# AnyiRao/video_unscreen

Measured on NVIDIA B200. Metric: frames/sec at 1080p & 4K (1/2/4/8 B200) + % HBM roofline vs host-CPU ref, higher is better.
Workload: dtype u8

## Files before the change

video_unscreen_b200/csrc/vu_median_sad.cuh:

```cuda
#pragma once
#include <cuda.h>
#include <cuda_runtime.h>
#include <stdint.h>

#include <type_traits>
#include "vu_tma.cuh"

namespace vu {
namespace msad {

__device__ __forceinline__ unsigned sad_acc(unsigned a, unsigned b, unsigned c) {
  unsigned d;
  asm("vabsdiff4.u32.u32.u32.add %0, %1, %2, %3;" : "=r"(d) : "r"(a), "r"(b), "r"(c));
  return d;
}

template <int G>
__device__ __forceinline__ void transpose_groups(unsigned (&d)[4 * G]) {
#pragma unroll
  for (int g = 0; g < G; ++g) {
    const unsigned a = d[4 * g], b = d[4 * g + 1], c = d[4 * g + 2], e = d[4 * g + 3];
    const unsigned ab_lo = __byte_perm(a, b, 0x5140), ab_hi = __byte_perm(a, b, 0x7362);
    const unsigned ce_lo = __byte_perm(c, e, 0x5140), ce_hi = __byte_perm(c, e, 0x7362);
    d[4 * g] = __byte_perm(ab_lo, ce_lo, 0x5410);
    d[4 * g + 1] = __byte_perm(ab_lo, ce_lo, 0x7632);
    d[4 * g + 2] = __byte_perm(ab_hi, ce_hi, 0x5410);
    d[4 * g + 3] = __byte_perm(ab_hi, ce_hi, 0x7632);
  }
}

template <int GI>
__device__ __forceinline__ unsigned ldg_strided(const uint8_t* base, unsigned stride) {
  unsigned long long addr;
  unsigned v;
  asm("mad.wide.u32 %0, %1, %2, %3;" : "=l"(addr) : "r"(stride), "n"(GI), "l"(base));
  asm volatile("ld.global.nc.u32 %0, [%1];" : "=r"(v) : "l"(addr));
  return v;
}

template <int I, int N, class F>
__device__ __forceinline__ void static_for(F&& f) {
  if constexpr (I < N) {
    f(std::integral_constant<int, I>{});
    static_for<I + 1, N>(f);
  }
}

constexpr unsigned BIG = 0x7fffffffu;
constexpr unsigned FULL = 0xffffffffu;

template <int SPLIT, int G, bool RANGE>
__device__ __forceinline__ void eval_s(const unsigned (&d)[4 * G], const int (&m)[4], int delta, unsigned (&S)[4]) {
  constexpr int LPS = 32 / SPLIT;
  unsigned q[4], s[4];
#pragma unroll
  for (int j = 0; j < 4; ++j) {
    q[j] = (unsigned)(RANGE ? min(max(m[j], 0), 255) : m[j]) * 0x01010101u;
    s[j] = 0;
  }
#pragma unroll
  for (int g = 0; g < G; ++g) {
#pragma unroll
    for (int j = 0; j < 4; ++j) s[j] = sad_acc(d[4 * g + j], q[j], s[j]);
  }
#pragma unroll
  for (int j = 0; j < 4; ++j) {
#pragma unroll
    for (int o = LPS; o < 32; o <<= 1) s[j] += __shfl_xor_sync(FULL, s[j], o);
    s[j] += (unsigned)(delta * m[j]);
    S[j] = (RANGE && (m[j] < 0 || m[j] > 255)) ? BIG : s[j];
  }
}

template <int SPLIT, int G, bool RANGE>
__device__ __forceinline__ void fib_search(const unsigned (&d)[4 * G], int delta, int k0, int fa, int fb, int fc, int (&a)[4], int (&r)[4],
                                           unsigned (&smin)[4], unsigned (&sl)[4], unsigned (&sr)[4]) {
  unsigned S1[4], S2[4];
  {
    int i1[4], i2[4];
#pragma unroll
    for (int j = 0; j < 4; ++j) {
      i1[j] = a[j] + fb;
      i2[j] = a[j] + fa;
      sl[j] = sr[j] = BIG;
    }
    eval_s<SPLIT, G, RANGE>(d, i1, delta, S1);
    eval_s<SPLIT, G, RANGE>(d, i2, delta, S2);
  }
#pragma unroll 1
  for (int k = k0; k >= 5; --k) {
    int nidx[4];
    bool left[4];
#pragma unroll
    for (int j = 0; j < 4; ++j) {
      left[j] = S1[j] <= S2[j];
      if (left[j]) {
        sr[j] = S2[j];
        S2[j] = S1[j];
        nidx[j] = a[j] + fc;
      } else {
        sl[j] = S1[j];
        a[j] += fb;
        S1[j] = S2[j];
        nidx[j] = a[j] + fb;
      }
    }
    unsigned Sn[4];
    eval_s<SPLIT, G, RANGE>(d, nidx, delta, Sn);
#pragma unroll
    for (int j = 0; j < 4; ++j) {
      if (left[j]) S1[j] = Sn[j];
      else S2[j] = Sn[j];
    }
    const int t = fb - fc;
    fa = fb;
    fb = fc;
    fc = t;
  }
#pragma unroll
  for (int j = 0; j < 4; ++j) {
    if (S1[j] <= S2[j]) {
      r[j] = a[j] + 1;
      smin[j] = S1[j];
      sr[j] = S2[j];
    } else {
      r[j] = a[j] + 2;
      smin[j] = S2[j];
      sl[j] = S1[j];
    }
  }
}

template <int SPLIT, int G, int SS>
__device__ __forceinline__ unsigned sad_median(const unsigned (&d)[4 * G], int n, int delta) {
  int a[4], r[4];
  unsigned smin[4], sl[4], sr[4];
  bool full = (SS == 0);
  if (SS > 0) {
    constexpr int EPP = 4 / SPLIT;
    const int part = (threadIdx.x & 31) / (32 / SPLIT);
    unsigned smp[EPP][4];
#pragma unroll
    for (int e = 0; e < EPP; ++e)
#pragma unroll
      for (int t = 0; t < 4; ++t) {
        unsigned v = d[4 * (t * SS) + e];
#pragma unroll
        for (int p = 1; p < SPLIT; ++p) v = (part == p) ? d[4 * (t * SS) + p * EPP + e] : v;
        smp[e][t] = v;
      }
    int est[EPP];
#pragma unroll
    for (int e = 0; e < EPP; ++e) est[e] = 0;
#pragma unroll 1
    for (int bit = 128; bit > 0; bit >>= 1) {
#pragma unroll
      for (int e = 0; e < EPP; ++e) {
        const unsigned q1 = (unsigned)(est[e] | bit) * 0x01010101u, q0 = q1 - 0x01010101u;
        unsigned s0 = 0, s1 = 0;
#pragma unroll
        for (int t = 0; t < 4; ++t) {
          s0 = sad_acc(smp[e][t], q0, s0);
          s1 = sad_acc(smp[e][t], q1, s1);
        }
        if (s1 < s0) est[e] |= bit;
      }
    }
#pragma unroll
    for (int j = 0; j < 4; ++j) {
      const int c = __shfl_sync(FULL, est[j % EPP], (j / EPP) * (32 / SPLIT) + (threadIdx.x & (32 / SPLIT - 1)));
      a[j] = min(max(c - 10, -1), 235);
    }
    fib_search<SPLIT, G, false>(d, delta, 8, 13, 8, 5, a, r, smin, sl, sr);
    bool fail = false;
#pragma unroll
    for (int j = 0; j < 4; ++j) fail |= (sl[j] == BIG && r[j] > 0) || (sr[j] == BIG && r[j] < 255);
    full = __any_sync(FULL, fail);
  }
  if (full) {
#pragma unroll
    for (int j = 0; j < 4; ++j) a[j] = -1;
    fib_search<SPLIT, G, true>(d, delta, 14, 233, 144, 89, a, r, smin, sl, sr);
  }
  int lo[4], hi[4];
#pragma unroll
  for (int j = 0; j < 4; ++j) lo[j] = hi[j] = r[j];
  if (!(n & 1)) {
    bool openL[4], openR[4];
    bool any = false;
#pragma unroll
    for (int j = 0; j < 4; ++j) {
      openL[j] = openR[j] = false;
      if (sl[j] == smin[j]) { lo[j] = r[j] - 1; openL[j] = lo[j] > 0; }
      if (sr[j] == smin[j]) { hi[j] = r[j] + 1; openR[j] = hi[j] < 255; }
      any |= openL[j] | openR[j];
    }
#pragma unroll 1
    for (int it = 0; it < 4 && __any_sync(FULL, any); ++it) {
      int idx[4];
      unsigned S[4];
#pragma unroll
      for (int j = 0; j < 4; ++j) idx[j] = openL[j] ? lo[j] - 1 : (openR[j] ? hi[j] + 1 : r[j]);
      eval_s<SPLIT, G, false>(d, idx, delta, S);
      any = false;
#pragma unroll
      for (int j = 0; j < 4; ++j) {
        if (openL[j]) {
          if (S[j] == smin[j]) { --lo[j]; openL[j] = lo[j] > 0; }
          else openL[j] = false;
        } else if (openR[j]) {
          if (S[j] == smin[j]) { ++hi[j]; openR[j] = hi[j] < 255; }
          else openR[j] = false;
        }
        any |= openL[j] | openR[j];
      }
    }
    if (__any_sync(FULL, any)) {
      int L[4], R[4];
#pragma unroll
      for (int j = 0; j < 4; ++j) { R[j] = lo[j]; L[j] = openL[j] ? 0 : lo[j]; }
      while (__any_sync(FULL, (L[0] < R[0]) | (L[1] < R[1]) | (L[2] < R[2]) | (L[3] < R[3]))) {
        int idx[4];
        unsigned S[4];
#pragma unroll
        for (int j = 0; j < 4; ++j) idx[j] = (L[j] + R[j]) >> 1;
        eval_s<SPLIT, G, false>(d, idx, delta, S);
#pragma unroll
        for (int j = 0; j < 4; ++j)
          if (L[j] < R[j]) {
            const int mid = (L[j] + R[j]) >> 1;
            if (S[j] == smin[j]) R[j] = mid;
            else L[j] = mid + 1;
          }
      }
#pragma unroll
      for (int j = 0; j < 4; ++j) { lo[j] = R[j]; L[j] = hi[j]; R[j] = openR[j] ? 255 : hi[j]; }
      while (__any_sync(FULL, (L[0] < R[0]) | (L[1] < R[1]) | (L[2] < R[2]) | (L[3] < R[3]))) {
        int idx[4];
        unsigned S[4];
#pragma unroll
        for (int j = 0; j < 4; ++j) idx[j] = (L[j] + R[j] + 1) >> 1;
        eval_s<SPLIT, G, false>(d, idx, delta, S);
#pragma unroll
        for (int j = 0; j < 4; ++j)
          if (L[j] < R[j]) {
            const int mid = (L[j] + R[j] + 1) >> 1;
            if (S[j] == smin[j]) L[j] = mid;
            else R[j] = mid - 1;
          }
      }
#pragma unroll
      for (int j = 0; j < 4; ++j) hi[j] = L[j];
    }
  }
  unsigned res = 0;
#pragma unroll
  for (int j = 0; j < 4; ++j) res |= (unsigned)((lo[j] + hi[j]) >> 1) << (8 * j);
  return res;
}

template <int SPLIT>
__device__ __forceinline__ bool pad_high(int part) { return SPLIT == 2 ? part == 1 : (part == 1 || part == 2); }

template <int SPLIT, int G, int GFULL, int SS, int CTAS>
__global__ void __launch_bounds__(128, CTAS) median_sad_kernel(const uint8_t* __restrict__ frames, uint8_t* __restrict__ out, int n, long long m,
                                                               int nseg, unsigned zero) {
  constexpr int LPS = 32 / SPLIT;
  constexpr int SEG = LPS * 4;
  const int lane = threadIdx.x & 31, warp = threadIdx.x >> 5;
  const int part = lane / LPS, li = lane % LPS;
  const int seg = blockIdx.x * 4 + warp;
  if (seg >= nseg) return;
  const int cnt0 = (n + SPLIT - 1) / SPLIT;
  const int cnt = (n - part + SPLIT - 1) / SPLIT;
  const int Q = (cnt0 + 3) >> 2;
  const unsigned pad = pad_high<SPLIT>(part) ? 0xFFFFFFFFu : 0u;
  int n0 = 0, n255 = 0;
#pragma unroll
  for (int p = 0; p < SPLIT; ++p) {
    const int c = 4 * G - (n - p + SPLIT - 1) / SPLIT;
    if (pad_high<SPLIT>(p)) n255 += c;
    else n0 += c;
  }
  const int delta = n255 - n0;
  unsigned gstride[4];
  const uint8_t* rowbase[4];
#pragma unroll
  for (int r = 0; r < 4; ++r) {
    rowbase[r] = frames + (long long)seg * SEG + li * 4 + ((long long)SPLIT * (r * Q) + part) * m;
    gstride[r] = (unsigned)(SPLIT * m) + (unsigned)r * zero;
  }
  unsigned d[4 * G];
  static_for<0, G>([&](auto gi) {
    constexpr int g = decltype(gi)::value;
#pragma unroll
    for (int r = 0; r < 4; ++r) {
      const bool ok = (r < 3 && g < GFULL) ? true : (g < Q && r * Q + g < cnt);
      d[4 * g + r] = pad;
      if (ok) d[4 * g + r] = ldg_strided<g>(rowbase[r], gstride[r]);
    }
  });
  transpose_groups<G>(d);
  const unsigned res = sad_median<SPLIT, G, SS>(d, n, delta);
  if (part == 0) reinterpret_cast<unsigned*>(out + (long long)seg * SEG)[li] = res;
}


using tma::mbar_expect_tx;
using tma::mbar_init;
using tma::mbar_wait;
__device__ __forceinline__ void tma_load_2d(unsigned dst, const void* tmap, int c0, int c1, unsigned mbar) { tma::load_2d(dst, tmap, c0, c1, mbar); }

template <int SPLIT, int G, int GQ, int SS, int WARPS, int CTAS>
__global__ void __launch_bounds__(WARPS * 32, CTAS) median_sad_tma_kernel(const __grid_constant__ CUtensorMap tmap, uint8_t* __restrict__ out, int n,
                                                                          int ntiles) {
  extern __shared__ __align__(128) uint8_t smem_tma[];
  constexpr int LPS = 32 / SPLIT;
  constexpr int SEG = LPS * 4;
  constexpr int TILE = WARPS * SEG;
  constexpr int ROWS = SPLIT * 4 * G;
  constexpr unsigned BOX_BYTES = 4 * G * TILE;
  const int lane = threadIdx.x & 31, warp = threadIdx.x >> 5;
  const int part = lane / LPS, li = lane % LPS;
  const int cnt0 = (n + SPLIT - 1) / SPLIT;
  const int Q = (cnt0 + 3) >> 2;
  const int delta = -(ROWS - n);
  uint64_t* mbar_p = reinterpret_cast<uint64_t*>(smem_tma + ROWS * TILE);
  unsigned* count_p = reinterpret_cast<unsigned*>(mbar_p + 1);
  const unsigned mbar = (unsigned)__cvta_generic_to_shared(mbar_p);
  const unsigned sdata = (unsigned)__cvta_generic_to_shared(smem_tma);
  auto fetch = [&](int tile) {
    mbar_expect_tx(mbar, SPLIT * BOX_BYTES);
#pragma unroll
    for (int b = 0; b < SPLIT; ++b) tma_load_2d(sdata + b * BOX_BYTES, &tmap, tile * (TILE > 256 ? TILE / 4 : TILE), b * 4 * G, mbar);
  };
  if (threadIdx.x == 0) {
    mbar_init(mbar, 1);
    *count_p = 0;
    asm volatile("fence.mbarrier_init.release.cluster;" ::: "memory");
  }
  __syncthreads();
  int tile = blockIdx.x;
  if (threadIdx.x == 0 && tile < ntiles) fetch(tile);
  const uint8_t* rowaddr[4];
#pragma unroll
  for (int r = 0; r < 4; ++r) rowaddr[r] = smem_tma + (SPLIT * (r * Q) + part) * TILE + warp * SEG + li * 4;
  unsigned parity = 0;
  for (; tile < ntiles; tile += gridDim.x) {
    mbar_wait(mbar, parity);
    parity ^= 1;
    unsigned d[4 * G];
#pragma unroll
    for (int g = 0; g < G; ++g) {
#pragma unroll
      for (int r = 0; r < 4; ++r) {
        d[4 * g + r] = 0;
        if (g < GQ || g < Q) d[4 * g + r] = *reinterpret_cast<const unsigned*>(rowaddr[r] + g * (SPLIT * TILE));
      }
    }
    transpose_groups<G>(d);
    __syncwarp();
    if (lane == 0) {
      __threadfence_block();
      const unsigned old = atomicAdd(count_p, 1u);
      if (old % WARPS == WARPS - 1 && tile + (int)gridDim.x < ntiles) {
        __threadfence_block();
        asm volatile("fence.proxy.async.shared::cta;" ::: "memory");
        fetch(tile + gridDim.x);
      }
    }
    const unsigned res = sad_median<SPLIT, G, SS>(d, n, delta);
    if (part == 0) reinterpret_cast<unsigned*>(out + ((long long)tile * WARPS + warp) * SEG)[li] = res;
  }
}

constexpr int RF_WARPS = 8, RF_ROWS = 64, RF_STAGES = 4, RF_PROBES = 8;
constexpr int RF_TILE = RF_WARPS * 64;
constexpr int RF_STAGE_BYTES = RF_ROWS * RF_TILE;
constexpr int RF_SMEM = RF_STAGES * RF_STAGE_BYTES + RF_STAGES * 16;

__global__ void __launch_bounds__(RF_WARPS * 32, 1) median_refine_kernel(const __grid_constant__ CUtensorMap tmap, uint8_t* __restrict__ out,
                                                                         uint8_t* __restrict__ flags, int n, int ntiles, int nchunks) {
  extern __shared__ __align__(128) uint8_t smem_rf[];
  const int lane = threadIdx.x & 31, warp = threadIdx.x >> 5;
  const int part = lane >> 4, li = lane & 15;
  uint64_t* mbar_p = reinterpret_cast<uint64_t*>(smem_rf + RF_STAGES * RF_STAGE_BYTES);
  unsigned* count_p = reinterpret_cast<unsigned*>(mbar_p + RF_STAGES);
  const unsigned mbar0 = (unsigned)__cvta_generic_to_shared(mbar_p);
  const unsigned sdata = (unsigned)__cvta_generic_to_shared(smem_rf);
  const int my_tiles = blockIdx.x < ntiles ? (ntiles - 1 - (int)blockIdx.x) / (int)gridDim.x + 1 : 0;
  const int J = my_tiles * nchunks;
  auto issue = [&](int j) {
    const int tile = blockIdx.x + (j / nchunks) * gridDim.x, chunk = j % nchunks, st = j % RF_STAGES;
    mbar_expect_tx(mbar0 + 8 * st, RF_STAGE_BYTES);
    tma_load_2d(sdata + st * RF_STAGE_BYTES, &tmap, tile * (RF_TILE / 4), chunk * RF_ROWS, mbar0 + 8 * st);
  };
  if (threadIdx.x == 0) {
    for (int st = 0; st < RF_STAGES; ++st) {
      mbar_init(mbar0 + 8 * st, 1);
      count_p[st] = 0;
    }
    asm volatile("fence.mbarrier_init.release.cluster;" ::: "memory");
  }
  __syncthreads();
  if (threadIdx.x == 0)
    for (int j = 0; j < RF_STAGES && j < J; ++j) issue(j);
  const int delta = -(nchunks * RF_ROWS - n);
  unsigned acc[RF_PROBES][4], q[RF_PROBES][4];
  int a0[4];
  const uint8_t* lane_row = smem_rf + part * RF_TILE + warp * 64 + li * 4;
  for (int j = 0; j < J; ++j) {
    const int tile = blockIdx.x + (j / nchunks) * gridDim.x, chunk = j % nchunks, st = j % RF_STAGES;
    const int64_t seg = (int64_t)tile * RF_WARPS + warp;
    if (chunk == 0) {
      const unsigned e = *reinterpret_cast<const unsigned*>(out + seg * 64 + li * 4);
#pragma unroll
      for (int k = 0; k < 4; ++k) {
        a0[k] = min(max((int)((e >> (8 * k)) & 255u) - 4, 0), 256 - RF_PROBES);
#pragma unroll
        for (int p = 0; p < RF_PROBES; ++p) {
          q[p][k] = (unsigned)(a0[k] + p) * 0x01010101u;
          acc[p][k] = 0u;
        }
      }
    }
// ... 57 lines not shown
```

video_unscreen_b200/csrc/vu_temporal.cu:

```cuda
#include <cstdlib>

#include "vu_common.cuh"
#include "vu_median_sad.cuh"

namespace vu {
namespace {

constexpr int WARPS = 7;
constexpr int MTHREADS = WARPS * 32;
constexpr int BIN_STRIDE = WARPS * 128;
constexpr int HIST_BYTES = 256 * BIN_STRIDE;

struct PolU16x2 {
  static constexpr int PX = 2;
  __device__ static __forceinline__ void add(unsigned char* base, unsigned w) {
#pragma unroll
    for (int j = 0; j < 2; ++j) atomicAdd(reinterpret_cast<unsigned*>(base + ((w >> (8 * j)) & 0xFFu) * BIN_STRIDE), 1u << (16 * j));
  }
  __device__ static __forceinline__ void unpack(unsigned w, unsigned* c) { c[0] = w & 0xFFFFu; c[1] = w >> 16; }
};

template <int PX>
__device__ __forceinline__ unsigned load_px(const uint8_t* p) {
  if (PX == 4) return __ldg(reinterpret_cast<const unsigned*>(p));
// ... 65 lines not shown
#pragma unroll
      for (int b = 0; b < 16; ++b) {
        unsigned t[PX];
        P::unpack(*reinterpret_cast<unsigned*>(base + (g * 16 + b) * BIN_STRIDE), t);
#pragma unroll
        for (int j = 0; j < PX; ++j) c[j] += t[j];
      }
#pragma unroll
      for (int j = 0; j < PX; ++j) {
        const unsigned nc = cum[j] + c[j];
        if (nc <= klo) { gsel[j][0] = g + 1; before[j][0] = nc; }
        if (nc <= khi) { gsel[j][1] = g + 1; before[j][1] = nc; }
        cum[j] = nc;
      }
    }
    unsigned res = 0;
#pragma unroll
    for (int j = 0; j < PX; ++j) {
      unsigned med[2];
#pragma unroll
      for (int q = 0; q < 2; ++q) {
        const unsigned k = q ? khi : klo;
        if (q == 1 && khi == klo) { med[1] = med[0]; continue; }
        const unsigned g = min(gsel[j][q], 15u);
        unsigned v = g * 16, c2 = before[j][q];
#pragma unroll 4
        for (int b = 0; b < 16; ++b) {
          unsigned t[PX];
          P::unpack(*reinterpret_cast<unsigned*>(base + (g * 16 + b) * BIN_STRIDE), t);
          c2 += t[j];
          if (c2 <= k) v = g * 16 + b + 1;
        }
        med[q] = min(v, 255u);
      }
      res |= ((med[0] + med[1]) >> 1) << (8 * j);
    }
    uint8_t* dst = out + (long long)seg * SEG;
    if (PX == 4) reinterpret_cast<unsigned*>(dst)[lane] = res;
    else reinterpret_cast<unsigned short*>(dst)[lane] = (unsigned short)res;
    __syncwarp();
  }
}

template <int SPLIT, int G, int GFULL, int SS, int CTAS>
int launch_median_sad(const uint8_t* frames, int n, int64_t m, int64_t nseg, uint8_t* out, vu_stream_t stream) {
  msad::median_sad_kernel<SPLIT, G, GFULL, SS, CTAS><<<(unsigned)((nseg + 3) / 4), 128, 0, S(stream)>>>(frames, out, n, m, (int)nseg, 0u);
  note_launch();
  return record_cuda(cudaGetLastError());
}

using tma::encode_tiled_fn;
using tma::EncodeTiledFn;

template <int SPLIT, int G, int GQ, int SS, int TMA_WARPS, int TMA_CTAS>
int launch_median_sad_tma(const uint8_t* frames, int n, int64_t m, int64_t ntiles, uint8_t* out, vu_stream_t stream, int64_t pitch = 0) {
  if (pitch == 0) pitch = m;
  constexpr int TILE = TMA_WARPS * (128 / SPLIT);
  constexpr int SMEM = SPLIT * 4 * G * TILE + 16;
  constexpr bool U32 = TILE > 256;
  static_assert(TILE <= 1024 && 4 * G <= 256, "TMA box limits");
  EncodeTiledFn enc = encode_tiled_fn();
  if (!enc) return VU_ERR_UNSUPPORTED;
  CUtensorMap tmap;
  const cuuint64_t dims[2] = {(cuuint64_t)(U32 ? m / 4 : m), (cuuint64_t)n};
  const cuuint64_t strides[1] = {(cuuint64_t)pitch};
  const cuuint32_t box[2] = {(cuuint32_t)(U32 ? TILE / 4 : TILE), (cuuint32_t)(4 * G)};
  const cuuint32_t estr[2] = {1, 1};
  if (enc(&tmap, U32 ? CU_TENSOR_MAP_DATA_TYPE_UINT32 : CU_TENSOR_MAP_DATA_TYPE_UINT8, 2, const_cast<uint8_t*>(frames), dims, strides, box, estr, CU_TENSOR_MAP_INTERLEAVE_NONE,
          CU_TENSOR_MAP_SWIZZLE_NONE, CU_TENSOR_MAP_L2_PROMOTION_L2_256B, CU_TENSOR_MAP_FLOAT_OOB_FILL_NONE) != CUDA_SUCCESS)
    return VU_ERR_UNSUPPORTED;
  auto kernel = msad::median_sad_tma_kernel<SPLIT, G, GQ, SS, TMA_WARPS, TMA_CTAS>;
  static bool configured = false;
  if (!configured) {
    int e = record_cuda(cudaFuncSetAttribute(kernel, cudaFuncAttributeMaxDynamicSharedMemorySize, SMEM));
    if (e) return e;
    configured = true;
  }
  const int64_t cap = (int64_t)device_sms() * TMA_CTAS;
  const int grid = (int)(ntiles < cap ? ntiles : cap);
  kernel<<<grid, TMA_WARPS * 32, SMEM, S(stream)>>>(tmap, out, n, (int)ntiles);
  note_launch();
  return record_cuda(cudaGetLastError());
}

__global__ void __launch_bounds__(256) median_tail_kernel(const uint8_t* __restrict__ frames, uint8_t* __restrict__ out, int n, long long m,
                                                          long long first) {
  __shared__ unsigned hist[256];
  const long long e = first + blockIdx.x;
  hist[threadIdx.x] = 0;
  __syncthreads();
  for (int f = threadIdx.x; f < n; f += 256) atomicAdd(&hist[__ldg(frames + (long long)f * m + e)], 1u);
  __syncthreads();
  if (threadIdx.x == 0) {
    const unsigned klo = (unsigned)(n - 1) >> 1, khi = (unsigned)n >> 1;
    unsigned cum = 0, lo = 255, hi = 255;
    bool flo = false, fhi = false;
    for (int b = 0; b < 256; ++b) {
      cum += hist[b];
      if (!flo && cum > klo) { lo = b; flo = true; }
      if (!fhi && cum > khi) { hi = b; fhi = true; }
    }
    out[e] = (uint8_t)((lo + hi) >> 1);
  }
}

constexpr int TT = 256;
__global__ void __launch_bounds__(TT) masked_mean_kernel(const uint8_t* __restrict__ frames, const uint8_t* __restrict__ masks, int n,
                                                         int64_t ngroups, int64_t npix, int min_count, uint8_t* __restrict__ bg_out,
                                                         uint8_t* __restrict__ always_out) {
  const int64_t stride = (int64_t)gridDim.x * blockDim.x;
  for (int64_t g = (int64_t)blockIdx.x * blockDim.x + threadIdx.x; g < ngroups; g += stride) {
    unsigned sum[12], cnt[4];
#pragma unroll
    for (int i = 0; i < 12; ++i) sum[i] = 0;
#pragma unroll
    for (int i = 0; i < 4; ++i) cnt[i] = 0;
    const unsigned* f4 = reinterpret_cast<const unsigned*>(frames) + 3 * g;
    const unsigned* m4 = reinterpret_cast<const unsigned*>(masks) + g;
    const int64_t fstride = npix * 3 / 4, mstride = npix / 4;
#pragma unroll 4
    for (int f = 0; f < n; ++f) {
      int c[12];
      unpack12(__ldg(f4), __ldg(f4 + 1), __ldg(f4 + 2), c);
      const unsigned mw = __ldg(m4);
      f4 += fstride;
      m4 += mstride;
#pragma unroll
      for (int i = 0; i < 4; ++i) {
        const unsigned mv = (mw >> (8 * i)) & 255u;
        const unsigned keep = 1u - mv / 255u;
        sum[3 * i] += c[3 * i] * keep;
        sum[3 * i + 1] += c[3 * i + 1] * keep;
        sum[3 * i + 2] += c[3 * i + 2] * keep;
// ... 187 lines not shown
        }
      }
    }
    if (f0 + MD_FPI < n) fetch_frames(f0 + MD_FPI);
  }
  if (!own) return;
  unsigned ow[6], aw[2] = {0u, 0u};
#pragma unroll
  for (int k = 0; k < 6; ++k) ow[k] = 0u;
  const unsigned walked = (unsigned)((n + MD_FPI - 1) / MD_FPI * MD_FPI);
#pragma unroll
  for (int i = 0; i < 8; ++i) {
    const unsigned c = walked - cnt[i];
    const bool always = c <= (unsigned)min_count;
    const double den = (double)(c ? c : 1u);
#pragma unroll
    for (int k = 0; k < 3; ++k) {
      const int b = 3 * i + k;
      const double q = fmin(fmax(__ddiv_rn((double)sum[b], den), 0.0), 255.0);
      ow[b >> 2] |= (always ? 0u : (unsigned)(int)q) << (8 * (b & 3));
    }
    aw[i >> 2] |= (always ? 255u : 0u) << (8 * (i & 3));
  }
  uint2* bo = reinterpret_cast<uint2*>(bg_out + ((int64_t)oy * w + ox) * 3);
#pragma unroll
  for (int k = 0; k < 3; ++k) bo[k] = make_uint2(ow[2 * k], ow[2 * k + 1]);
  *reinterpret_cast<uint2*>(always_out + (int64_t)oy * w + ox) = make_uint2(aw[0], aw[1]);
}

template <class P, int U>
int launch_median(const uint8_t* frames, int n, int64_t m, int64_t nseg, uint8_t* out, vu_stream_t stream, const uint8_t* flags = nullptr) {
  static bool configured = false;
  if (!configured) {
    int e = record_cuda(cudaFuncSetAttribute(median_kernel<P, U>, cudaFuncAttributeMaxDynamicSharedMemorySize, HIST_BYTES));
    if (e) return e;
    configured = true;
  }
  int grid = device_sms();
  const int64_t need = (nseg + WARPS - 1) / WARPS;
  if (need < grid) grid = (int)need;
  median_kernel<P, U><<<grid, MTHREADS, HIST_BYTES, S(stream)>>>(frames, out, n, m, (int)nseg, flags);
  note_launch();
  return record_cuda(cudaGetLastError());
}

int launch_median_two_pass(const uint8_t* frames, int n, int64_t m, int64_t nseg, uint8_t* out, uint8_t* flags, vu_stream_t stream) {
  EncodeTiledFn enc = encode_tiled_fn();
  if (!enc) return VU_ERR_UNSUPPORTED;
  const int64_t ntiles = nseg / msad::RF_WARPS;
  if (ntiles == 0 || ntiles > 0x7fffffff) return VU_ERR_UNSUPPORTED;
  const int step = (n + 303) / 304;
  const int nsub = (n + step - 1) / step;
  int e;
  if (nsub <= 152) e = launch_median_sad_tma<2, 19, 11, 2, 8, 2>(frames, nsub, m, ntiles, out, stream, (int64_t)step * m);
  else if (nsub <= 232) e = launch_median_sad_tma<2, 29, 20, 5, 8, 1>(frames, nsub, m, ntiles, out, stream, (int64_t)step * m);
  else e = launch_median_sad_tma<2, 38, 30, 8, 8, 1>(frames, nsub, m, ntiles, out, stream, (int64_t)step * m);
  if (e) return e;
  CUtensorMap tmap;
  const cuuint64_t dims[2] = {(cuuint64_t)(m / 4), (cuuint64_t)n};
  const cuuint64_t strides[1] = {(cuuint64_t)m};
  const cuuint32_t box[2] = {(cuuint32_t)(msad::RF_TILE / 4), (cuuint32_t)msad::RF_ROWS};
  const cuuint32_t estr[2] = {1, 1};
  if (enc(&tmap, CU_TENSOR_MAP_DATA_TYPE_UINT32, 2, const_cast<uint8_t*>(frames), dims, strides, box, estr, CU_TENSOR_MAP_INTERLEAVE_NONE,
          CU_TENSOR_MAP_SWIZZLE_NONE, CU_TENSOR_MAP_L2_PROMOTION_L2_256B, CU_TENSOR_MAP_FLOAT_OOB_FILL_NONE) != CUDA_SUCCESS)
    return VU_ERR_UNSUPPORTED;
  static bool configured = false;
  if (!configured) {
    e = record_cuda(cudaFuncSetAttribute(msad::median_refine_kernel, cudaFuncAttributeMaxDynamicSharedMemorySize, msad::RF_SMEM));
    if (e) return e;
    configured = true;
  }
  const int nchunks = (n + msad::RF_ROWS - 1) / msad::RF_ROWS;
  const int grid = (int)(ntiles < device_sms() ? ntiles : device_sms());
  msad::median_refine_kernel<<<grid, msad::RF_WARPS * 32, msad::RF_SMEM, S(stream)>>>(tmap, out, flags, n, (int)ntiles, nchunks);
  note_launch();
  e = record_cuda(cudaGetLastError());
  if (e) return e;
  const int64_t done = ntiles * msad::RF_WARPS;
  if (done < nseg) {
    e = record_cuda(cudaMemsetAsync(flags + done, 1, (size_t)(nseg - done), S(stream)));
    if (e) return e;
  }
  return launch_median<PolU16x2, 32>(frames, n, m, nseg, out, stream, flags);
}

}
}

using namespace vu;

static const bool g_median_direct = [] {
  const char* e = getenv("VU_MEDIAN_DIRECT");
  return e && atoi(e) != 0;
}();

extern "C" size_t vu_temporal_median_workspace_bytes(int n, int64_t m) { return (n > 608 && m > 0) ? (size_t)(m / 64 + 64) : 0; }

extern "C" int vu_temporal_median_u8(const uint8_t* frames, int n, int64_t m, uint8_t* out, vu_stream_t stream) {
  return vu_temporal_median_u8_ws(frames, n, m, out, nullptr, 0, stream);
}

extern "C" int vu_temporal_median_u8_ws(const uint8_t* frames, int n, int64_t m, uint8_t* out, void* workspace, size_t workspace_bytes,
                                        vu_stream_t stream) {
  VU_REQUIRE(frames && out && m >= 0);
  if (n < 1 || n > 65535) return VU_ERR_UNSUPPORTED;
  if (m == 0) return VU_OK;
  const bool fits32 = m < (1ll << 30);
  const int path = (n <= 304 && fits32) ? 0 : ((n <= 608 && fits32) ? 1 : 2);
  const int seg = path == 0 ? 64 : (path == 1 ? 32 : 64);
  const int align = path == 2 ? 2 : 4;
  const bool ok = (reinterpret_cast<uintptr_t>(frames) % align == 0) && (reinterpret_cast<uintptr_t>(out) % align == 0) && (m % align == 0);
  int64_t nseg = ok ? m / seg : 0;
  if (nseg > 0x7fffffff) return VU_ERR_UNSUPPORTED;
  int64_t tiled = 0;
  if (nseg > 0) {
    int e;
    const bool al16 = (reinterpret_cast<uintptr_t>(frames) % 16 == 0) && (m % 16 == 0);
    const int64_t ntiles = nseg / 8;
    if (al16 && path != 2 && n > 80 && ntiles > 0 && !g_median_direct) {
      if (n <= 152) e = launch_median_sad_tma<2, 19, 11, 2, 8, 2>(frames, n, m, ntiles, out, stream);
      else if (n <= 232) e = launch_median_sad_tma<2, 29, 20, 5, 8, 1>(frames, n, m, ntiles, out, stream);
      else if (n <= 304) e = launch_median_sad_tma<2, 38, 30, 8, 8, 1>(frames, n, m, ntiles, out, stream);
      else if (n <= 464) e = launch_median_sad_tma<4, 29, 20, 5, 8, 1>(frames, n, m, ntiles, out, stream);
      else e = launch_median_sad_tma<4, 38, 30, 8, 8, 1>(frames, n, m, ntiles, out, stream);
      if (e == VU_OK) {
        const int64_t done = ntiles * 8;
        frames += done * seg;
        out += done * seg;
        nseg -= done;
        tiled = done * seg;
      } else if (e != VU_ERR_UNSUPPORTED) {
        return e;
      }
    }
    if (nseg == 0) {
      e = VU_OK;
    } else if (path == 0) {
      if (n <= 80) e = launch_median_sad<2, 10, 0, 0, 4>(frames, n, m, nseg, out, stream);
      else if (n <= 152) e = launch_median_sad<2, 19, 11, 2, 4>(frames, n, m, nseg, out, stream);
      else if (n <= 232) e = launch_median_sad<2, 29, 20, 5, 2>(frames, n, m, nseg, out, stream);
      else e = launch_median_sad<2, 38, 30, 8, 2>(frames, n, m, nseg, out, stream);
    } else if (path == 1) {
      e = n <= 464 ? launch_median_sad<4, 29, 20, 5, 2>(frames, n, m, nseg, out, stream) : launch_median_sad<4, 38, 30, 8, 2>(frames, n, m, nseg, out, stream);
    } else {
      e = VU_ERR_UNSUPPORTED;
      if (workspace && workspace_bytes >= vu_temporal_median_workspace_bytes(n, m) && al16 && m < (1ll << 32) && !g_median_direct)
        e = launch_median_two_pass(frames, n, m, nseg, out, static_cast<uint8_t*>(workspace), stream);
      if (e == VU_ERR_UNSUPPORTED) e = launch_median<PolU16x2, 32>(frames, n, m, nseg, out, stream);
    }
    if (e) return e;
  }
  const int64_t first = nseg * seg;
  const int64_t rem = m - tiled;
  if (first < rem) {
    if (rem - first > 0x7fffffff) return VU_ERR_UNSUPPORTED;
    median_tail_kernel<<<(unsigned)(rem - first), 256, 0, S(stream)>>>(frames, out, n, m, first);
    note_launch();
    return record_cuda(cudaGetLastError());
  }
  return VU_OK;
}

extern "C" int vu_masked_temporal_mean_dilate32(const uint8_t* frames, const uint8_t* masks, int n, int h, int w, int min_count, uint8_t* bg_out,
                                                uint8_t* mask_always_out, vu_stream_t stream) {
  VU_REQUIRE(frames && masks && bg_out && mask_always_out && n >= 1 && h > 0 && w > 0);
  if (n > 16000000) return VU_ERR_UNSUPPORTED;
  const void* ptrs[] = {frames, masks, bg_out, mask_always_out};
  for (const void* p : ptrs)
    if (reinterpret_cast<uintptr_t>(p) & 15) return VU_ERR_UNSUPPORTED;
  if (w % 16 != 0 || (h + MD_TH - 1) / MD_TH > 65535) return VU_ERR_UNSUPPORTED;
  dim3 grid((w + MD_TW - 1) / MD_TW, (h + MD_TH - 1) / MD_TH);
  masked_mean_dilate_kernel<<<grid, 256, 0, S(stream)>>>(frames, masks, n, h, w, min_count, bg_out, mask_always_out);
  VU_RETURN_LAUNCH();
}

extern "C" int vu_masked_temporal_mean(const uint8_t* frames, const uint8_t* masks, int n, int64_t npix, int min_count, uint8_t* bg_out,
                                       uint8_t* mask_always_out, vu_stream_t stream) {
// ... 19 lines not shown
```

Measured before the change: 831,500.

## Load median tiles via swizzled 3D TMA and ldmatrix transpose instead of scalar LDS

Switches the TMA median kernel to a 3D tensor map with 128B swizzle and reads each frame column block with ldmatrix .trans, which produces pixel-major byte words directly instead of scalar shared loads followed by a byte-permute transpose. The SAD median search is generalised to E elements per thread with configurable shuffle-reduction masks and split accumulators, so each thread now handles 2 pixels over 2*G words. This is meant to cut shared-memory load and transpose overhead and the ILP bottleneck in the SAD chain. In exchange it relies on the b8 ldmatrix m16n16 form, and it changes the pixels-per-thread split and the tile config table.

```diff
diff --git a/video_unscreen_b200/csrc/vu_median_sad.cuh b/video_unscreen_b200/csrc/vu_median_sad.cuh
--- a/video_unscreen_b200/csrc/vu_median_sad.cuh
+++ b/video_unscreen_b200/csrc/vu_median_sad.cuh
@@ -49,50 +49,60 @@
 constexpr unsigned BIG = 0x7fffffffu;
 constexpr unsigned FULL = 0xffffffffu;
 
-template <int SPLIT, int G, bool RANGE>
-__device__ __forceinline__ void eval_s(const unsigned (&d)[4 * G], const int (&m)[4], int delta, unsigned (&S)[4]) {
-  constexpr int LPS = 32 / SPLIT;
-  unsigned q[4], s[4];
-#pragma unroll
-  for (int j = 0; j < 4; ++j) {
+__host__ __device__ constexpr int lowest_bit(unsigned x) { return x & 1u ? 0 : 1 + lowest_bit(x >> 1); }
+template <unsigned XMASK>
+__host__ __device__ constexpr int parts_of() { return XMASK ? (int)(XMASK >> lowest_bit(XMASK)) + 1 : 1; }
+
+template <int E, unsigned XMASK, int K, bool RANGE>
+__device__ __forceinline__ void eval_s(const unsigned (&d)[E * K], const int (&m)[E], int delta, unsigned (&S)[E]) {
+  constexpr int NA = E < 4 ? 4 / E : 1;
+  static_assert(K % NA == 0, "words per element must split evenly over the accumulators");
+  unsigned q[E], s[E][NA];
+#pragma unroll
+  for (int j = 0; j < E; ++j) {
     q[j] = (unsigned)(RANGE ? min(max(m[j], 0), 255) : m[j]) * 0x01010101u;
-    s[j] = 0;
-  }
-#pragma unroll
-  for (int g = 0; g < G; ++g) {
-#pragma unroll
-    for (int j = 0; j < 4; ++j) s[j] = sad_acc(d[4 * g + j], q[j], s[j]);
-  }
-#pragma unroll
-  for (int j = 0; j < 4; ++j) {
-#pragma unroll
-    for (int o = LPS; o < 32; o <<= 1) s[j] += __shfl_xor_sync(FULL, s[j], o);
-    s[j] += (unsigned)(delta * m[j]);
-    S[j] = (RANGE && (m[j] < 0 || m[j] > 255)) ? BIG : s[j];
-  }
-}
-
-template <int SPLIT, int G, bool RANGE>
-__device__ __forceinline__ void fib_search(const unsigned (&d)[4 * G], int delta, int k0, int fa, int fb, int fc, int (&a)[4], int (&r)[4],
-                                           unsigned (&smin)[4], unsigned (&sl)[4], unsigned (&sr)[4]) {
-  unsigned S1[4], S2[4];
+#pragma unroll
+    for (int a = 0; a < NA; ++a) s[j][a] = 0;
+  }
+#pragma unroll
+  for (int k = 0; k < K; ++k) {
+#pragma unroll
+    for (int j = 0; j < E; ++j) s[j][k % NA] = sad_acc(d[E * k + j], q[j], s[j][k % NA]);
+  }
+#pragma unroll
+  for (int j = 0; j < E; ++j) {
+    unsigned t = s[j][0];
+#pragma unroll
+    for (int a = 1; a < NA; ++a) t += s[j][a];
+#pragma unroll
+    for (int o = 1; o < 32; o <<= 1)
+      if (XMASK & o) t += __shfl_xor_sync(FULL, t, o);
+    t += (unsigned)(delta * m[j]);
+    S[j] = (RANGE && (m[j] < 0 || m[j] > 255)) ? BIG : t;
+  }
+}
+
+template <int E, unsigned XMASK, int K, bool RANGE>
+__device__ __forceinline__ void fib_search(const unsigned (&d)[E * K], int delta, int k0, int fa, int fb, int fc, int (&a)[E], int (&r)[E],
+                                           unsigned (&smin)[E], unsigned (&sl)[E], unsigned (&sr)[E]) {
+  unsigned S1[E], S2[E];
   {
-    int i1[4], i2[4];
-#pragma unroll
-    for (int j = 0; j < 4; ++j) {
+    int i1[E], i2[E];
+#pragma unroll
+    for (int j = 0; j < E; ++j) {
       i1[j] = a[j] + fb;
       i2[j] = a[j] + fa;
       sl[j] = sr[j] = BIG;
     }
-    eval_s<SPLIT, G, RANGE>(d, i1, delta, S1);
-    eval_s<SPLIT, G, RANGE>(d, i2, delta, S2);
+    eval_s<E, XMASK, K, RANGE>(d, i1, delta, S1);
+    eval_s<E, XMASK, K, RANGE>(d, i2, delta, S2);
   }
 #pragma unroll 1
   for (int k = k0; k >= 5; --k) {
-    int nidx[4];
-    bool left[4];
-#pragma unroll
-    for (int j = 0; j < 4; ++j) {
+    int nidx[E];
+    bool left[E];
+#pragma unroll
+    for (int j = 0; j < E; ++j) {
       left[j] = S1[j] <= S2[j];
       if (left[j]) {
         sr[j] = S2[j];
@@ -105,10 +115,10 @@
         nidx[j] = a[j] + fb;
       }
     }
-    unsigned Sn[4];
-    eval_s<SPLIT, G, RANGE>(d, nidx, delta, Sn);
-#pragma unroll
-    for (int j = 0; j < 4; ++j) {
+    unsigned Sn[E];
+    eval_s<E, XMASK, K, RANGE>(d, nidx, delta, Sn);
+#pragma unroll
+    for (int j = 0; j < E; ++j) {
       if (left[j]) S1[j] = Sn[j];
       else S2[j] = Sn[j];
     }
@@ -118,7 +128,7 @@
     fc = t;
   }
 #pragma unroll
-  for (int j = 0; j < 4; ++j) {
+  for (int j = 0; j < E; ++j) {
     if (S1[j] <= S2[j]) {
       r[j] = a[j] + 1;
       smin[j] = S1[j];
@@ -131,22 +141,33 @@
   }
 }
 
-template <int SPLIT, int G, int SS>
-__device__ __forceinline__ unsigned sad_median(const unsigned (&d)[4 * G], int n, int delta) {
-  int a[4], r[4];
-  unsigned smin[4], sl[4], sr[4];
+template <int E>
+__device__ __forceinline__ bool open_any(const int (&L)[E], const int (&R)[E]) {
+  bool o = false;
+#pragma unroll
+  for (int j = 0; j < E; ++j) o |= L[j] < R[j];
+  return o;
+}
+
+template <int E, unsigned XMASK, int K, int SS>
+__device__ __forceinline__ unsigned sad_median(const unsigned (&d)[E * K], int n, int delta) {
+  int a[E], r[E];
+  unsigned smin[E], sl[E], sr[E];
   bool full = (SS == 0);
   if (SS > 0) {
-    constexpr int EPP = 4 / SPLIT;
-    const int part = (threadIdx.x & 31) / (32 / SPLIT);
+    constexpr int PARTS = parts_of<XMASK>();
+    constexpr int PSHIFT = XMASK ? lowest_bit(XMASK) : 0;
+    constexpr int EPP = E / PARTS;
+    const int lane = threadIdx.x & 31;
+    const int part = (lane & XMASK) >> PSHIFT;
     unsigned smp[EPP][4];
 #pragma unroll
     for (int e = 0; e < EPP; ++e)
 #pragma unroll
       for (int t = 0; t < 4; ++t) {
-        unsigned v = d[4 * (t * SS) + e];
-#pragma unroll
-        for (int p = 1; p < SPLIT; ++p) v = (part == p) ? d[4 * (t * SS) + p * EPP + e] : v;
+        unsigned v = d[E * (t * SS) + e];
+#pragma unroll
+        for (int p = 1; p < PARTS; ++p) v = (part == p) ? d[E * (t * SS) + p * EPP + e] : v;
         smp[e][t] = v;
       }
     int est[EPP];
@@ -167,29 +188,29 @@
       }
     }
 #pragma unroll
-    for (int j = 0; j < 4; ++j) {
-      const int c = __shfl_sync(FULL, est[j % EPP], (j / EPP) * (32 / SPLIT) + (threadIdx.x & (32 / SPLIT - 1)));
+    for (int j = 0; j < E; ++j) {
+      const int c = PARTS == 1 ? est[j] : __shfl_sync(FULL, est[j % EPP], (lane & ~XMASK) | ((j / EPP) << PSHIFT));
       a[j] = min(max(c - 10, -1), 235);
     }
-    fib_search<SPLIT, G, false>(d, delta, 8, 13, 8, 5, a, r, smin, sl, sr);
+    fib_search<E, XMASK, K, false>(d, delta, 8, 13, 8, 5, a, r, smin, sl, sr);
     bool fail = false;
 #pragma unroll
-    for (int j = 0; j < 4; ++j) fail |= (sl[j] == BIG && r[j] > 0) || (sr[j] == BIG && r[j] < 255);
+    for (int j = 0; j < E; ++j) fail |= (sl[j] == BIG && r[j] > 0) || (sr[j] == BIG && r[j] < 255);
     full = __any_sync(FULL, fail);
   }
   if (full) {
 #pragma unroll
-    for (int j = 0; j < 4; ++j) a[j] = -1;
-    fib_search<SPLIT, G, true>(d, delta, 14, 233, 144, 89, a, r, smin, sl, sr);
-  }
-  int lo[4], hi[4];
-#pragma unroll
-  for (int j = 0; j < 4; ++j) lo[j] = hi[j] = r[j];
+    for (int j = 0; j < E; ++j) a[j] = -1;
+    fib_search<E, XMASK, K, true>(d, delta, 14, 233, 144, 89, a, r, smin, sl, sr);
+  }
+  int lo[E], hi[E];
+#pragma unroll
+  for (int j = 0; j < E; ++j) lo[j] = hi[j] = r[j];
   if (!(n & 1)) {
-    bool openL[4], openR[4];
+    bool openL[E], openR[E];
     bool any = false;
 #pragma unroll
-    for (int j = 0; j < 4; ++j) {
+    for (int j = 0; j < E; ++j) {
       openL[j] = openR[j] = false;
       if (sl[j] == smin[j]) { lo[j] = r[j] - 1; openL[j] = lo[j] > 0; }
       if (sr[j] == smin[j]) { hi[j] = r[j] + 1; openR[j] = hi[j] < 255; }
@@ -197,14 +218,14 @@
     }
 #pragma unroll 1
     for (int it = 0; it < 4 && __any_sync(FULL, any); ++it) {
-      int idx[4];
-      unsigned S[4];
-#pragma unroll
-      for (int j = 0; j < 4; ++j) idx[j] = openL[j] ? lo[j] - 1 : (openR[j] ? hi[j] + 1 : r[j]);
-      eval_s<SPLIT, G, false>(d, idx, delta, S);
+      int idx[E];
+      unsigned S[E];
+#pragma unroll
+      for (int j = 0; j < E; ++j) idx[j] = openL[j] ? lo[j] - 1 : (openR[j] ? hi[j] + 1 : r[j]);
+      eval_s<E, XMASK, K, false>(d, idx, delta, S);
       any = false;
 #pragma unroll
-      for (int j = 0; j < 4; ++j) {
+      for (int j = 0; j < E; ++j) {
         if (openL[j]) {
           if (S[j] == smin[j]) { --lo[j]; openL[j] = lo[j] > 0; }
           else openL[j] = false;
@@ -216,17 +237,17 @@
       }
     }
     if (__any_sync(FULL, any)) {
-      int L[4], R[4];
-#pragma unroll
-      for (int j = 0; j < 4; ++j) { R[j] = lo[j]; L[j] = openL[j] ? 0 : lo[j]; }
-      while (__any_sync(FULL, (L[0] < R[0]) | (L[1] < R[1]) | (L[2] < R[2]) | (L[3] < R[3]))) {
-        int idx[4];
-        unsigned S[4];
-#pragma unroll
-        for (int j = 0; j < 4; ++j) idx[j] = (L[j] + R[j]) >> 1;
-        eval_s<SPLIT, G, false>(d, idx, delta, S);
-#pragma unroll
-        for (int j = 0; j < 4; ++j)
+      int L[E], R[E];
+#pragma unroll
+      for (int j = 0; j < E; ++j) { R[j] = lo[j]; L[j] = openL[j] ? 0 : lo[j]; }
+      while (__any_sync(FULL, open_any(L, R))) {
+        int idx[E];
+        unsigned S[E];
+#pragma unroll
+        for (int j = 0; j < E; ++j) idx[j] = (L[j] + R[j]) >> 1;
+        eval_s<E, XMASK, K, false>(d, idx, delta, S);
+#pragma unroll
+        for (int j = 0; j < E; ++j)
           if (L[j] < R[j]) {
             const int mid = (L[j] + R[j]) >> 1;
             if (S[j] == smin[j]) R[j] = mid;
@@ -234,15 +255,15 @@
           }
       }
 #pragma unroll
-      for (int j = 0; j < 4; ++j) { lo[j] = R[j]; L[j] = hi[j]; R[j] = openR[j] ? 255 : hi[j]; }
-      while (__any_sync(FULL, (L[0] < R[0]) | (L[1] < R[1]) | (L[2] < R[2]) | (L[3] < R[3]))) {
-        int idx[4];
-        unsigned S[4];
-#pragma unroll
-        for (int j = 0; j < 4; ++j) idx[j] = (L[j] + R[j] + 1) >> 1;
-        eval_s<SPLIT, G, false>(d, idx, delta, S);
-#pragma unroll
-        for (int j = 0; j < 4; ++j)
+      for (int j = 0; j < E; ++j) { lo[j] = R[j]; L[j] = hi[j]; R[j] = openR[j] ? 255 : hi[j]; }
+      while (__any_sync(FULL, open_any(L, R))) {
+        int idx[E];
+        unsigned S[E];
+#pragma unroll
+        for (int j = 0; j < E; ++j) idx[j] = (L[j] + R[j] + 1) >> 1;
+        eval_s<E, XMASK, K, false>(d, idx, delta, S);
+#pragma unroll
+        for (int j = 0; j < E; ++j)
           if (L[j] < R[j]) {
             const int mid = (L[j] + R[j] + 1) >> 1;
             if (S[j] == smin[j]) L[j] = mid;
@@ -250,12 +271,12 @@
           }
       }
 #pragma unroll
-      for (int j = 0; j < 4; ++j) hi[j] = L[j];
+      for (int j = 0; j < E; ++j) hi[j] = L[j];
     }
   }
   unsigned res = 0;
 #pragma unroll
-  for (int j = 0; j < 4; ++j) res |= (unsigned)((lo[j] + hi[j]) >> 1) << (8 * j);
+  for (int j = 0; j < E; ++j) res |= (unsigned)((lo[j] + hi[j]) >> 1) << (8 * j);
   return res;
 }
 
@@ -301,7 +322,7 @@
     }
   });
   transpose_groups<G>(d);
-  const unsigned res = sad_median<SPLIT, G, SS>(d, n, delta);
+  const unsigned res = sad_median<4, 32u - LPS, G, SS>(d, n, delta);
   if (part == 0) reinterpret_cast<unsigned*>(out + (long long)seg * SEG)[li] = res;
 }
 
@@ -311,28 +332,42 @@
 using tma::mbar_wait;
 __device__ __forceinline__ void tma_load_2d(unsigned dst, const void* tmap, int c0, int c1, unsigned mbar) { tma::load_2d(dst, tmap, c0, c1, mbar); }
 
-template <int SPLIT, int G, int GQ, int SS, int WARPS, int CTAS>
+__device__ __forceinline__ void ldsm_x2_trans(unsigned addr, unsigned& r0, unsigned& r1, unsigned& r2, unsigned& r3) {
+  asm volatile("ldmatrix.sync.aligned.m16n16.x2.trans.shared.b8 {%0, %1, %2, %3}, [%4];" : "=r"(r0), "=r"(r1), "=r"(r2), "=r"(r3) : "r"(addr) : "memory");
+}
+
+template <int C, int G, int WARPS>
+struct TmaTile {
+  static_assert(C == 2 || C == 4, "a warp owns 2 or 4 column blocks of 16 bytes");
+  static constexpr int P = 4 / C;
+  static constexpr int SEG = 16 * C;
+  static constexpr int TILE = WARPS * SEG;
+  static constexpr int COLS = TILE / 128;
+  static constexpr int ROWS = 8 * P * G;
+  static constexpr int row_boxes(int b) { return (ROWS % b == 0 && (ROWS / b) % 8 == 0 && ROWS / b <= 256) ? b : row_boxes(b + 1); }
+  static constexpr int BOX_ROWS = ROWS / row_boxes(1);
+  static constexpr int BYTES = ROWS * TILE;
+  static constexpr int SMEM = BYTES + 1024 + 16;
+  static_assert(TILE % 128 == 0, "whole 128-byte columns");
+};
+
+template <int C, int G, int SS, int WARPS, int CTAS>
 __global__ void __launch_bounds__(WARPS * 32, CTAS) median_sad_tma_kernel(const __grid_constant__ CUtensorMap tmap, uint8_t* __restrict__ out, int n,
                                                                           int ntiles) {
-  extern __shared__ __align__(128) uint8_t smem_tma[];
-  constexpr int LPS = 32 / SPLIT;
-  constexpr int SEG = LPS * 4;
-  constexpr int TILE = WARPS * SEG;
-  constexpr int ROWS = SPLIT * 4 * G;
-  constexpr unsigned BOX_BYTES = 4 * G * TILE;
+  extern __shared__ __align__(1024) uint8_t smem_tma[];
+  using T = TmaTile<C, G, WARPS>;
+  constexpr unsigned XMASK = 3u & ~(unsigned)(C - 1);
   const int lane = threadIdx.x & 31, warp = threadIdx.x >> 5;
-  const int part = lane / LPS, li = lane % LPS;
-  const int cnt0 = (n + SPLIT - 1) / SPLIT;
-  const int Q = (cnt0 + 3) >> 2;
-  const int delta = -(ROWS - n);
-  uint64_t* mbar_p = reinterpret_cast<uint64_t*>(smem_tma + ROWS * TILE);
+  const int delta = -(T::ROWS - n);
+  const unsigned sraw = (unsigned)__cvta_generic_to_shared(smem_tma);
+  const unsigned sdata = (sraw + 1023u) & ~1023u;
+  uint64_t* mbar_p = reinterpret_cast<uint64_t*>(smem_tma + (sdata - sraw) + T::BYTES);
   unsigned* count_p = reinterpret_cast<unsigned*>(mbar_p + 1);
   const unsigned mbar = (unsigned)__cvta_generic_to_shared(mbar_p);
-  const unsigned sdata = (unsigned)__cvta_generic_to_shared(smem_tma);
   auto fetch = [&](int tile) {
-    mbar_expect_tx(mbar, SPLIT * BOX_BYTES);
-#pragma unroll
-    for (int b = 0; b < SPLIT; ++b) tma_load_2d(sdata + b * BOX_BYTES, &tmap, tile * (TILE > 256 ? TILE / 4 : TILE), b * 4 * G, mbar);
+    mbar_expect_tx(mbar, T::BYTES);
+#pragma unroll
+    for (int r = 0; r < T::ROWS; r += T::BOX_ROWS) tma::load_3d(sdata + r * T::TILE, &tmap, 0, tile * T::COLS, r, mbar);
   };
   if (threadIdx.x == 0) {
     mbar_init(mbar, 1);
@@ -342,23 +377,23 @@
   __syncthreads();
   int tile = blockIdx.x;
   if (threadIdx.x == 0 && tile < ntiles) fetch(tile);
-  const uint8_t* rowaddr[4];
-#pragma unroll
-  for (int r = 0; r < 4; ++r) rowaddr[r] = smem_tma + (SPLIT * (r * Q) + part) * TILE + warp * SEG + li * 4;
+  unsigned laddr;
+  {
+    const int rho = lane & 15, M = lane >> 4, qq = rho >> 2;
+    const int f0 = 8 * (qq / C) + 4 * ((M ^ qq) & 1) + (rho & 3);
+    const int byte = warp * T::SEG + 16 * (qq % C);
+    const int unit = f0 * T::COLS + (byte >> 7);
+    laddr = sdata + unit * 128 + ((((byte >> 4) & 7) ^ (unit & 7)) << 4);
+  }
+  const int q = lane & 3;
+  const int ebyte = warp * T::SEG + 16 * (q % C) + (lane >> 2);
   unsigned parity = 0;
   for (; tile < ntiles; tile += gridDim.x) {
     mbar_wait(mbar, parity);
     parity ^= 1;
     unsigned d[4 * G];
 #pragma unroll
-    for (int g = 0; g < G; ++g) {
-#pragma unroll
-      for (int r = 0; r < 4; ++r) {
-        d[4 * g + r] = 0;
-        if (g < GQ || g < Q) d[4 * g + r] = *reinterpret_cast<const unsigned*>(rowaddr[r] + g * (SPLIT * TILE));
-      }
-    }
-    transpose_groups<G>(d);
+    for (int j = 0; j < G; ++j) ldsm_x2_trans(laddr + j * (8 * T::P * T::TILE), d[4 * j], d[4 * j + 1], d[4 * j + 2], d[4 * j + 3]);
     __syncwarp();
     if (lane == 0) {
       __threadfence_block();
@@ -369,8 +404,12 @@
         fetch(tile + gridDim.x);
       }
     }
-    const unsigned res = sad_median<SPLIT, G, SS>(d, n, delta);
-    if (part == 0) reinterpret_cast<unsigned*>(out + ((long long)tile * WARPS + warp) * SEG)[li] = res;
+    const unsigned res = sad_median<2, XMASK, 2 * G, SS>(d, n, delta);
+    if (q < C) {
+      uint8_t* o = out + (long long)tile * T::TILE + ebyte;
+      o[0] = (uint8_t)res;
+      o[8] = (uint8_t)(res >> 8);
+    }
   }
 }
 
diff --git a/video_unscreen_b200/csrc/vu_temporal.cu b/video_unscreen_b200/csrc/vu_temporal.cu
--- a/video_unscreen_b200/csrc/vu_temporal.cu
+++ b/video_unscreen_b200/csrc/vu_temporal.cu
@@ -141,33 +141,32 @@
 using tma::encode_tiled_fn;
 using tma::EncodeTiledFn;
 
-template <int SPLIT, int G, int GQ, int SS, int TMA_WARPS, int TMA_CTAS>
+template <int C, int G, int SS, int TMA_WARPS, int TMA_CTAS>
 int launch_median_sad_tma(const uint8_t* frames, int n, int64_t m, int64_t ntiles, uint8_t* out, vu_stream_t stream, int64_t pitch = 0) {
+  using T = msad::TmaTile<C, G, TMA_WARPS>;
+  static_assert(8 % TMA_WARPS == 0, "tiles of whole fractions of 8 segments");
+  ntiles *= 8 / TMA_WARPS;
   if (pitch == 0) pitch = m;
-  constexpr int TILE = TMA_WARPS * (128 / SPLIT);
-  constexpr int SMEM = SPLIT * 4 * G * TILE + 16;
-  constexpr bool U32 = TILE > 256;
-  static_assert(TILE <= 1024 && 4 * G <= 256, "TMA box limits");
   EncodeTiledFn enc = encode_tiled_fn();
   if (!enc) return VU_ERR_UNSUPPORTED;
   CUtensorMap tmap;
-  const cuuint64_t dims[2] = {(cuuint64_t)(U32 ? m / 4 : m), (cuuint64_t)n};
-  const cuuint64_t strides[1] = {(cuuint64_t)pitch};
-  const cuuint32_t box[2] = {(cuuint32_t)(U32 ? TILE / 4 : TILE), (cuuint32_t)(4 * G)};
-  const cuuint32_t estr[2] = {1, 1};
-  if (enc(&tmap, U32 ? CU_TENSOR_MAP_DATA_TYPE_UINT32 : CU_TENSOR_MAP_DATA_TYPE_UINT8, 2, const_cast<uint8_t*>(frames), dims, strides, box, estr, CU_TENSOR_MAP_INTERLEAVE_NONE,
-          CU_TENSOR_MAP_SWIZZLE_NONE, CU_TENSOR_MAP_L2_PROMOTION_L2_256B, CU_TENSOR_MAP_FLOAT_OOB_FILL_NONE) != CUDA_SUCCESS)
+  const cuuint64_t dims[3] = {32, (cuuint64_t)(m / 128), (cuuint64_t)n};
+  const cuuint64_t strides[2] = {128, (cuuint64_t)pitch};
+  const cuuint32_t box[3] = {32, (cuuint32_t)T::COLS, (cuuint32_t)T::BOX_ROWS};
+  const cuuint32_t estr[3] = {1, 1, 1};
+  if (enc(&tmap, CU_TENSOR_MAP_DATA_TYPE_UINT32, 3, const_cast<uint8_t*>(frames), dims, strides, box, estr, CU_TENSOR_MAP_INTERLEAVE_NONE,
+          CU_TENSOR_MAP_SWIZZLE_128B, CU_TENSOR_MAP_L2_PROMOTION_L2_256B, CU_TENSOR_MAP_FLOAT_OOB_FILL_NONE) != CUDA_SUCCESS)
     return VU_ERR_UNSUPPORTED;
-  auto kernel = msad::median_sad_tma_kernel<SPLIT, G, GQ, SS, TMA_WARPS, TMA_CTAS>;
+  auto kernel = msad::median_sad_tma_kernel<C, G, SS, TMA_WARPS, TMA_CTAS>;
   static bool configured = false;
   if (!configured) {
-    int e = record_cuda(cudaFuncSetAttribute(kernel, cudaFuncAttributeMaxDynamicSharedMemorySize, SMEM));
+    int e = record_cuda(cudaFuncSetAttribute(kernel, cudaFuncAttributeMaxDynamicSharedMemorySize, T::SMEM));
     if (e) return e;
     configured = true;
   }
   const int64_t cap = (int64_t)device_sms() * TMA_CTAS;
   const int grid = (int)(ntiles < cap ? ntiles : cap);
-  kernel<<<grid, TMA_WARPS * 32, SMEM, S(stream)>>>(tmap, out, n, (int)ntiles);
+  kernel<<<grid, TMA_WARPS * 32, T::SMEM, S(stream)>>>(tmap, out, n, (int)ntiles);
   note_launch();
   return record_cuda(cudaGetLastError());
 }
@@ -461,9 +460,9 @@
   const int step = (n + 303) / 304;
   const int nsub = (n + step - 1) / step;
   int e;
-  if (nsub <= 152) e = launch_median_sad_tma<2, 19, 11, 2, 8, 2>(frames, nsub, m, ntiles, out, stream, (int64_t)step * m);
-  else if (nsub <= 232) e = launch_median_sad_tma<2, 29, 20, 5, 8, 1>(frames, nsub, m, ntiles, out, stream, (int64_t)step * m);
-  else e = launch_median_sad_tma<2, 38, 30, 8, 8, 1>(frames, nsub, m, ntiles, out, stream, (int64_t)step * m);
+  if (nsub <= 152) e = launch_median_sad_tma<4, 19, 6, 8, 2>(frames, nsub, m, ntiles, out, stream, (int64_t)step * m);
+  else if (nsub <= 232) e = launch_median_sad_tma<4, 29, 12, 8, 1>(frames, nsub, m, ntiles, out, stream, (int64_t)step * m);
+  else e = launch_median_sad_tma<4, 38, 19, 8, 1>(frames, nsub, m, ntiles, out, stream, (int64_t)step * m);
   if (e) return e;
   CUtensorMap tmap;
   const cuuint64_t dims[2] = {(cuuint64_t)(m / 4), (cuuint64_t)n};
@@ -527,11 +526,11 @@
     const bool al16 = (reinterpret_cast<uintptr_t>(frames) % 16 == 0) && (m % 16 == 0);
     const int64_t ntiles = nseg / 8;
     if (al16 && path != 2 && n > 80 && ntiles > 0 && !g_median_direct) {
-      if (n <= 152) e = launch_median_sad_tma<2, 19, 11, 2, 8, 2>(frames, n, m, ntiles, out, stream);
-      else if (n <= 232) e = launch_median_sad_tma<2, 29, 20, 5, 8, 1>(frames, n, m, ntiles, out, stream);
-      else if (n <= 304) e = launch_median_sad_tma<2, 38, 30, 8, 8, 1>(frames, n, m, ntiles, out, stream);
-      else if (n <= 464) e = launch_median_sad_tma<4, 29, 20, 5, 8, 1>(frames, n, m, ntiles, out, stream);
-      else e = launch_median_sad_tma<4, 38, 30, 8, 8, 1>(frames, n, m, ntiles, out, stream);
+      if (n <= 152) e = launch_median_sad_tma<4, 19, 6, 8, 2>(frames, n, m, ntiles, out, stream);
+      else if (n <= 232) e = launch_median_sad_tma<4, 29, 12, 8, 1>(frames, n, m, ntiles, out, stream);
+      else if (n <= 304) e = launch_median_sad_tma<4, 38, 19, 8, 1>(frames, n, m, ntiles, out, stream);
+      else if (n <= 464) e = launch_median_sad_tma<2, 29, 12, 8, 1>(frames, n, m, ntiles, out, stream);
+      else e = launch_median_sad_tma<2, 38, 19, 8, 1>(frames, n, m, ntiles, out, stream);
       if (e == VU_OK) {
         const int64_t done = ntiles * 8;
         frames += done * seg;
```

Result: faster. 905,100 (median of 6 runs) (+8.8%).
